# cgtuebingen/3D-RE-GEN

Hardware: NVIDIA H100
Metric: objects->mesh/sec (256^3 SDF, 50 DiT steps) (higher is better)
Workload: dtype f16

## Files before the change

### 3d-re-gen_b200/csrc/attn.cu

```cuda
#include <cuda_fp16.h>
#include <math.h>

#include "r3g_internal.h"
#include "r3g_ptx.cuh"

namespace {

using namespace r3g;

constexpr int kD = 64;
constexpr int kWG = 3;
constexpr int kBQ = 64 * kWG;
constexpr int kBKV = 128;
constexpr int kStg = 3;
constexpr int kQBytes = 64 * kD * 2;
constexpr int kTileBytes = kBKV * kD * 2;
constexpr int kTilesBytes = kQBytes * kWG + 2 * kStg * kTileBytes;
constexpr int kSmemBytes = kTilesBytes + 1024 + 256;
constexpr int kThreads = 128 * kWG + 32;

struct AttnParams {
  __half* o;
  int64_t o_sb, o_sh, o_sl;
  int Lq, Lk;
  float scale_log2;
};

__global__ void __launch_bounds__(kThreads, 1)
attention_kernel(const __grid_constant__ CUtensorMap tmap_q, const __grid_constant__ CUtensorMap tmap_k,
                 const __grid_constant__ CUtensorMap tmap_v, const AttnParams p) {
  extern __shared__ uint8_t smem_raw[];
  uint8_t* smem = reinterpret_cast<uint8_t*>((reinterpret_cast<uintptr_t>(smem_raw) + 1023) & ~(uintptr_t)1023);
  uint8_t* sQ = smem;
  uint8_t* sK = sQ + kWG * kQBytes;
  uint8_t* sV = sK + kStg * kTileBytes;
  uint64_t* q_full = reinterpret_cast<uint64_t*>(smem + kTilesBytes);
  uint64_t* k_full = q_full + 1;
  uint64_t* v_full = k_full + kStg;
  uint64_t* k_empty = v_full + kStg;
  uint64_t* v_empty = k_empty + kStg;

  const int warp = threadIdx.x >> 5;
  const int lane = threadIdx.x & 31;
  const int q0 = blockIdx.x * kBQ;
  const int h = blockIdx.y, b = blockIdx.z;
  const int n_kv = (p.Lk + kBKV - 1) / kBKV;

  if (warp == 4 * kWG && lane == 0) {
    tma_prefetch_desc(&tmap_q);
    tma_prefetch_desc(&tmap_k);
    tma_prefetch_desc(&tmap_v);
    mbar_init(q_full, 1);
    for (int s = 0; s < kStg; ++s) {
      mbar_init(&k_full[s], 1);
      mbar_init(&v_full[s], 1);
      mbar_init(&k_empty[s], 128 * kWG);
      mbar_init(&v_empty[s], 128 * kWG);
    }
    fence_barrier_init();
  }
  __syncthreads();
  pdl_wait();

  if (warp == 4 * kWG) {
    if (lane == 0) {
      const int groups = min(kWG, (p.Lq - q0 + 63) / 64);
      mbar_expect_tx(q_full, groups * kQBytes);
      for (int g = 0; g < groups; ++g) tma_load_4d(sQ + g * kQBytes, &tmap_q, q_full, 0, q0 + 64 * g, h, b, kEvictFirst);
      for (int j = 0; j < n_kv; ++j) {
        const int st = j % kStg;
        const uint32_t ph = (j / kStg) & 1;
        mbar_wait(&k_empty[st], ph ^ 1);
        mbar_expect_tx(&k_full[st], kTileBytes);
        tma_load_4d(sK + st * kTileBytes, &tmap_k, &k_full[st], 0, j * kBKV, h, b, kEvictLast);
        mbar_wait(&v_empty[st], ph ^ 1);
        mbar_expect_tx(&v_full[st], kTileBytes);
        tma_load_4d(sV + st * kTileBytes, &tmap_v, &v_full[st], 0, j * kBKV, h, b, kEvictLast);
      }
    }
    return;
  }

  const int wg = warp >> 2;
  const int r0 = (warp & 3) * 16 + (lane >> 2);
  const int c0 = 2 * (lane & 3);
  const uint32_t aq = smem_u32(sQ + wg * kQBytes);
  float o[kD / 2];
#pragma unroll
  for (int i = 0; i < kD / 2; ++i) o[i] = 0.f;
  float m_run[2] = {-INFINITY, -INFINITY}, l_run[2] = {0.f, 0.f};
  mbar_wait(q_full, 0);
  for (int j = 0; j < n_kv; ++j) {
    const int st = j % kStg;
    const uint32_t ph = (j / kStg) & 1;
    float s[kBKV / 2];
    mbar_wait(&k_full[st], ph);
    const uint32_t ak = smem_u32(sK + st * kTileBytes);
    wgmma_fence();
#pragma unroll
    for (int k = 0; k < kD / 16; ++k)
      wgmma_m64n128k16_ss(s, gmma_desc_sw128(aq + k * 32, 1024, 16), gmma_desc_sw128(ak + k * 32, 1024, 16),
                          k ? 1u : 0u);
    wgmma_commit();
    wgmma_wait<0>();
    wgmma_reg_fence<kBKV / 2>(s);
    mbar_arrive(&k_empty[st]);

    const int valid = min(kBKV, p.Lk - j * kBKV);
    if (valid < kBKV) {
#pragma unroll
      for (int i = 0; i < kBKV / 2; ++i)
        if (8 * (i >> 2) + c0 + (i & 1) >= valid) s[i] = -INFINITY;
    }
    float mx[2] = {-INFINITY, -INFINITY};
#pragma unroll
    for (int i = 0; i < kBKV / 2; ++i) mx[(i >> 1) & 1] = fmaxf(mx[(i >> 1) & 1], s[i]);
    float alpha[2];
#pragma unroll
    for (int rr = 0; rr < 2; ++rr) {
      mx[rr] = fmaxf(mx[rr], __shfl_xor_sync(0xffffffffu, mx[rr], 1));
      mx[rr] = fmaxf(mx[rr], __shfl_xor_sync(0xffffffffu, mx[rr], 2));
      const float m_new = fmaxf(m_run[rr], mx[rr] * p.scale_log2);
      alpha[rr] = ex2_approx(m_run[rr] - m_new);
      m_run[rr] = m_new;
      l_run[rr] *= alpha[rr];
    }
#pragma unroll
    for (int i = 0; i < kD / 2; ++i) o[i] *= alpha[(i >> 1) & 1];
    uint32_t pk[kBKV / 16][4];
#pragma unroll
    for (int i = 0; i < kBKV / 2; i += 2) {
      const int rr = (i >> 1) & 1;
      const float e0 = ex2_approx(fmaf(s[i], p.scale_log2, -m_run[rr]));
      const float e1 = ex2_approx(fmaf(s[i + 1], p.scale_log2, -m_run[rr]));
      l_run[rr] += e0 + e1;
      pk[i >> 3][(i >> 1) & 3] = pack_half2(e0, e1);
    }
    mbar_wait(&v_full[st], ph);
    const uint32_t av = smem_u32(sV + st * kTileBytes);
    wgmma_fence();
#pragma unroll
    for (int k = 0; k < kBKV / 16; ++k) wgmma_m64n64k16_rs_tb(o, pk[k], gmma_desc_sw128(av + k * 2048, 1024, 1024), 1u);
    wgmma_commit();
    wgmma_wait<0>();
    wgmma_reg_fence<kD / 2>(o);
    mbar_arrive(&v_empty[st]);
  }

  float inv_l[2];
#pragma unroll
  for (int rr = 0; rr < 2; ++rr) {
    float l = l_run[rr];
    l += __shfl_xor_sync(0xffffffffu, l, 1);
    l += __shfl_xor_sync(0xffffffffu, l, 2);
    inv_l[rr] = 1.f / l;
  }
#pragma unroll
  for (int rr = 0; rr < 2; ++rr) {
    const int qrow = q0 + wg * 64 + r0 + 8 * rr;
    if (qrow >= p.Lq) continue;
    __half* op = p.o + (int64_t)b * p.o_sb + (int64_t)h * p.o_sh + (int64_t)qrow * p.o_sl;
#pragma unroll
    for (int i = 2 * rr; i < kD / 2; i += 4)
      *reinterpret_cast<uint32_t*>(op + 8 * (i >> 2) + c0) = pack_half2(o[i] * inv_l[rr], o[i + 1] * inv_l[rr]);
  }
}

int make_qkv_map(r3g_ctx* ctx, CUtensorMap* m, const void* base, int64_t sb, int64_t sh, int64_t sl, int B, int H,
                 int L, int box_rows) {
  const uint64_t dims[4] = {(uint64_t)kD, (uint64_t)L, (uint64_t)H, (uint64_t)B};
  const uint64_t strides[4] = {2, (uint64_t)sl * 2, (uint64_t)sh * 2, (uint64_t)sb * 2};
  const uint32_t box[4] = {(uint32_t)kD, (uint32_t)box_rows, 1, 1};
  return r3g_make_tmap_f16(ctx, m, base, 4, dims, strides, box);
}

}

extern "C" int r3g_attention(r3g_ctx* ctx, const r3g_attention_args* a, void* stream) {
  R3G_ENTRY(ctx, "attention");
  if (!a || !a->q || !a->k || !a->v || !a->o) return r3g_fail(ctx, R3G_E_INVALID, "attention: null argument");
  if (a->B < 1 || a->H < 1 || a->Lq < 1 || a->Lk < 1) return r3g_fail(ctx, R3G_E_INVALID, "attention: empty shape");
  if (a->o_sl % 8 || a->o_sh % 8 || a->o_sb % 8 || !r3g_aligned16(a->o))
    return r3g_fail(ctx, R3G_E_INVALID, "attention: output strides must be multiples of 8 halfs");
  CUtensorMap mq, mk, mv;
  int rc;
  if ((rc = make_qkv_map(ctx, &mq, a->q, a->q_sb, a->q_sh, a->q_sl, a->B, a->H, a->Lq, 64))) return rc;
  if ((rc = make_qkv_map(ctx, &mk, a->k, a->k_sb, a->k_sh, a->k_sl, a->B, a->H, a->Lk, kBKV))) return rc;
  if ((rc = make_qkv_map(ctx, &mv, a->v, a->v_sb, a->v_sh, a->v_sl, a->B, a->H, a->Lk, kBKV))) return rc;
  AttnParams p;
  p.o = (__half*)a->o;
  p.o_sb = a->o_sb; p.o_sh = a->o_sh; p.o_sl = a->o_sl;
  p.Lq = a->Lq; p.Lk = a->Lk;
  p.scale_log2 = a->scale * 1.4426950408889634f;
  if (!(ctx->attr_done & R3G_ATTR_ATTENTION)) {
    R3G_CUDA_OK(ctx, cudaFuncSetAttribute(attention_kernel, cudaFuncAttributeMaxDynamicSharedMemorySize, kSmemBytes));
    R3G_CUDA_OK(ctx, cudaFuncSetAttribute(attention_kernel, cudaFuncAttributePreferredSharedMemoryCarveout, 100));
    ctx->attr_done |= R3G_ATTR_ATTENTION;
  }
  dim3 grid((a->Lq + kBQ - 1) / kBQ, a->H, a->B);
  R3G_CUDA_OK(ctx, r3g_launch_pdl(ctx, attention_kernel, grid, dim3(kThreads), kSmemBytes, (cudaStream_t)stream, mq, mk, mv, p));
  R3G_LAUNCH_OK(ctx);
  return R3G_OK;
}
```

### 3d-re-gen_b200/csrc/r3g_ptx.cuh

```cuda
#pragma once
#include <cuda.h>
#include <cuda_fp16.h>
#include <cuda_runtime.h>
#include <stdint.h>

namespace r3g {

__device__ __forceinline__ uint32_t smem_u32(const void* p) {
  return static_cast<uint32_t>(__cvta_generic_to_shared(p));
}

__device__ __forceinline__ bool elect_one() {
  uint32_t pred = 0;
  asm volatile(
      "{\n\t.reg .pred P;\n\t"
      "elect.sync _|P, 0xffffffff;\n\t"
      "selp.u32 %0, 1, 0, P;\n\t}\n"
      : "=r"(pred));
  return pred != 0;
}

__device__ __forceinline__ void mbar_init(uint64_t* bar, uint32_t count) {
  asm volatile("mbarrier.init.shared::cta.b64 [%0], %1;\n" ::"r"(smem_u32(bar)), "r"(count));
}
__device__ __forceinline__ void pdl_wait() { asm volatile("griddepcontrol.wait;" ::: "memory"); }
__device__ __forceinline__ void pdl_trigger() { asm volatile("griddepcontrol.launch_dependents;" ::: "memory"); }

__device__ __forceinline__ void fence_barrier_init() {
  asm volatile("fence.mbarrier_init.release.cluster;\n" ::: "memory");
}
__device__ __forceinline__ void mbar_expect_tx(uint64_t* bar, uint32_t bytes) {
  asm volatile("mbarrier.arrive.expect_tx.shared::cta.b64 _, [%0], %1;\n" ::"r"(smem_u32(bar)), "r"(bytes)
               : "memory");
}
__device__ __forceinline__ void mbar_arrive(uint64_t* bar) {
  asm volatile("mbarrier.arrive.shared::cta.b64 _, [%0];\n" ::"r"(smem_u32(bar)) : "memory");
}
constexpr uint32_t kMbarSuspendHint = 0x989680u;
__device__ __forceinline__ bool mbar_try_wait(uint64_t* bar, uint32_t parity) {
  uint32_t ok;
  asm volatile(
      "{\n\t.reg .pred P;\n\t"
      "mbarrier.try_wait.parity.shared::cta.b64 P, [%1], %2, %3;\n\t"
      "selp.u32 %0, 1, 0, P;\n\t}\n"
      : "=r"(ok)
      : "r"(smem_u32(bar)), "r"(parity), "r"(kMbarSuspendHint)
      : "memory");
  return ok != 0;
}
__device__ __forceinline__ void mbar_wait(uint64_t* bar, uint32_t parity) {
  while (!mbar_try_wait(bar, parity)) {
  }
}

__device__ __forceinline__ void fence_proxy_async_smem() {
  asm volatile("fence.proxy.async.shared::cta;\n" ::: "memory");
}

__device__ __forceinline__ void named_bar_sync(uint32_t id, uint32_t count) {
  asm volatile("bar.sync %0, %1;\n" ::"r"(id), "r"(count) : "memory");
}

__device__ __forceinline__ void tma_prefetch_desc(const CUtensorMap* m) {
  asm volatile("prefetch.tensormap [%0];\n" ::"l"(reinterpret_cast<uint64_t>(m)) : "memory");
}
constexpr uint64_t kEvictNormal = 0x1000000000000000ull;
constexpr uint64_t kEvictFirst = 0x12F0000000000000ull;
constexpr uint64_t kEvictLast = 0x14F0000000000000ull;

__device__ __forceinline__ void tma_load_2d(void* smem_dst, const CUtensorMap* m, uint64_t* bar, int c0, int c1,
                                            uint64_t hint = kEvictNormal) {
  asm volatile(
      "cp.async.bulk.tensor.2d.shared::cluster.global.mbarrier::complete_tx::bytes.L2::cache_hint"
      " [%0], [%1, {%3, %4}], [%2], %5;\n" ::"r"(smem_u32(smem_dst)),
      "l"(reinterpret_cast<uint64_t>(m)), "r"(smem_u32(bar)), "r"(c0), "r"(c1), "l"(hint)
      : "memory");
}
__device__ __forceinline__ void tma_load_3d(void* smem_dst, const CUtensorMap* m, uint64_t* bar, int c0, int c1,
                                            int c2, uint64_t hint = kEvictNormal) {
  asm volatile(
      "cp.async.bulk.tensor.3d.shared::cluster.global.mbarrier::complete_tx::bytes.L2::cache_hint"
      " [%0], [%1, {%3, %4, %5}], [%2], %6;\n" ::"r"(smem_u32(smem_dst)),
      "l"(reinterpret_cast<uint64_t>(m)), "r"(smem_u32(bar)), "r"(c0), "r"(c1), "r"(c2), "l"(hint)
      : "memory");
}
__device__ __forceinline__ void tma_load_4d(void* smem_dst, const CUtensorMap* m, uint64_t* bar, int c0, int c1,
                                            int c2, int c3, uint64_t hint = kEvictNormal) {
  asm volatile(
      "cp.async.bulk.tensor.4d.shared::cluster.global.mbarrier::complete_tx::bytes.L2::cache_hint"
      " [%0], [%1, {%3, %4, %5, %6}], [%2], %7;\n" ::"r"(smem_u32(smem_dst)),
      "l"(reinterpret_cast<uint64_t>(m)), "r"(smem_u32(bar)), "r"(c0), "r"(c1), "r"(c2), "r"(c3), "l"(hint)
      : "memory");
}

__device__ __forceinline__ void wgmma_fence() { asm volatile("wgmma.fence.sync.aligned;\n" ::: "memory"); }
__device__ __forceinline__ void wgmma_commit() { asm volatile("wgmma.commit_group.sync.aligned;\n" ::: "memory"); }
template <int N>
__device__ __forceinline__ void wgmma_wait() {
  asm volatile("wgmma.wait_group.sync.aligned %0;\n" ::"n"(N) : "memory");
}
template <int N>
__device__ __forceinline__ void wgmma_reg_fence(float* d) {
#pragma unroll
  for (int i = 0; i < N; ++i) asm volatile("" : "+f"(d[i])::"memory");
}
__device__ __forceinline__ void wgmma_m64n128k16_ss(float* d, uint64_t desc_a, uint64_t desc_b, uint32_t accumulate) {
  asm volatile(
      "{\n\t.reg .pred p;\n\t"
      "setp.ne.b32 p, %66, 0;\n\t"
      "wgmma.mma_async.sync.aligned.m64n128k16.f32.f16.f16 "
      "{%0, %1, %2, %3, %4, %5, %6, %7, %8, %9, %10, %11, %12, %13, %14, %15, %16, %17, %18, %19, %20, %21, %22, %23, %24, %25, %26, %27, %28, %29, %30, %31, %32, %33, %34, %35, %36, %37, %38, %39, %40, %41, %42, %43, %44, %45, %46, %47, %48, %49, %50, %51, %52, %53, %54, %55, %56, %57, %58, %59, %60, %61, %62, %63}, "
      "%64, %65, p, 1, 1, 0, 0;\n\t}\n"
      : "+f"(d[0]), "+f"(d[1]), "+f"(d[2]), "+f"(d[3]), "+f"(d[4]), "+f"(d[5]), "+f"(d[6]), "+f"(d[7]), "+f"(d[8]), "+f"(d[9]), "+f"(d[10]), "+f"(d[11]), "+f"(d[12]), "+f"(d[13]), "+f"(d[14]), "+f"(d[15]), "+f"(d[16]), "+f"(d[17]), "+f"(d[18]), "+f"(d[19]), "+f"(d[20]), "+f"(d[21]), "+f"(d[22]), "+f"(d[23]), "+f"(d[24]), "+f"(d[25]), "+f"(d[26]), "+f"(d[27]), "+f"(d[28]), "+f"(d[29]), "+f"(d[30]), "+f"(d[31]), "+f"(d[32]), "+f"(d[33]), "+f"(d[34]), "+f"(d[35]), "+f"(d[36]), "+f"(d[37]), "+f"(d[38]), "+f"(d[39]), "+f"(d[40]), "+f"(d[41]), "+f"(d[42]), "+f"(d[43]), "+f"(d[44]), "+f"(d[45]), "+f"(d[46]), "+f"(d[47]), "+f"(d[48]), "+f"(d[49]), "+f"(d[50]), "+f"(d[51]), "+f"(d[52]), "+f"(d[53]), "+f"(d[54]), "+f"(d[55]), "+f"(d[56]), "+f"(d[57]), "+f"(d[58]), "+f"(d[59]), "+f"(d[60]), "+f"(d[61]), "+f"(d[62]), "+f"(d[63])
      : "l"(desc_a), "l"(desc_b), "r"(accumulate));
}
__device__ __forceinline__ void wgmma_m64n256k16_ss(float* d, uint64_t desc_a, uint64_t desc_b, uint32_t accumulate) {
  asm volatile(
      "{\n\t.reg .pred p;\n\t"
      "setp.ne.b32 p, %130, 0;\n\t"
      "wgmma.mma_async.sync.aligned.m64n256k16.f32.f16.f16 "
      "{%0, %1, %2, %3, %4, %5, %6, %7, %8, %9, %10, %11, %12, %13, %14, %15, %16, %17, %18, %19, %20, %21, %22, %23, %24, %25, %26, %27, %28, %29, %30, %31, %32, %33, %34, %35, %36, %37, %38, %39, %40, %41, %42, %43, %44, %45, %46, %47, %48, %49, %50, %51, %52, %53, %54, %55, %56, %57, %58, %59, %60, %61, %62, %63, %64, %65, %66, %67, %68, %69, %70, %71, %72, %73, %74, %75, %76, %77, %78, %79, %80, %81, %82, %83, %84, %85, %86, %87, %88, %89, %90, %91, %92, %93, %94, %95, %96, %97, %98, %99, %100, %101, %102, %103, %104, %105, %106, %107, %108, %109, %110, %111, %112, %113, %114, %115, %116, %117, %118, %119, %120, %121, %122, %123, %124, %125, %126, %127}, "
      "%128, %129, p, 1, 1, 0, 0;\n\t}\n"
      : "+f"(d[0]), "+f"(d[1]), "+f"(d[2]), "+f"(d[3]), "+f"(d[4]), "+f"(d[5]), "+f"(d[6]), "+f"(d[7]), "+f"(d[8]), "+f"(d[9]), "+f"(d[10]), "+f"(d[11]), "+f"(d[12]), "+f"(d[13]), "+f"(d[14]), "+f"(d[15]), "+f"(d[16]), "+f"(d[17]), "+f"(d[18]), "+f"(d[19]), "+f"(d[20]), "+f"(d[21]), "+f"(d[22]), "+f"(d[23]), "+f"(d[24]), "+f"(d[25]), "+f"(d[26]), "+f"(d[27]), "+f"(d[28]), "+f"(d[29]), "+f"(d[30]), "+f"(d[31]), "+f"(d[32]), "+f"(d[33]), "+f"(d[34]), "+f"(d[35]), "+f"(d[36]), "+f"(d[37]), "+f"(d[38]), "+f"(d[39]), "+f"(d[40]), "+f"(d[41]), "+f"(d[42]), "+f"(d[43]), "+f"(d[44]), "+f"(d[45]), "+f"(d[46]), "+f"(d[47]), "+f"(d[48]), "+f"(d[49]), "+f"(d[50]), "+f"(d[51]), "+f"(d[52]), "+f"(d[53]), "+f"(d[54]), "+f"(d[55]), "+f"(d[56]), "+f"(d[57]), "+f"(d[58]), "+f"(d[59]), "+f"(d[60]), "+f"(d[61]), "+f"(d[62]), "+f"(d[63]), "+f"(d[64]), "+f"(d[65]), "+f"(d[66]), "+f"(d[67]), "+f"(d[68]), "+f"(d[69]), "+f"(d[70]), "+f"(d[71]), "+f"(d[72]), "+f"(d[73]), "+f"(d[74]), "+f"(d[75]), "+f"(d[76]), "+f"(d[77]), "+f"(d[78]), "+f"(d[79]), "+f"(d[80]), "+f"(d[81]), "+f"(d[82]), "+f"(d[83]), "+f"(d[84]), "+f"(d[85]), "+f"(d[86]), "+f"(d[87]), "+f"(d[88]), "+f"(d[89]), "+f"(d[90]), "+f"(d[91]), "+f"(d[92]), "+f"(d[93]), "+f"(d[94]), "+f"(d[95]), "+f"(d[96]), "+f"(d[97]), "+f"(d[98]), "+f"(d[99]), "+f"(d[100]), "+f"(d[101]), "+f"(d[102]), "+f"(d[103]), "+f"(d[104]), "+f"(d[105]), "+f"(d[106]), "+f"(d[107]), "+f"(d[108]), "+f"(d[109]), "+f"(d[110]), "+f"(d[111]), "+f"(d[112]), "+f"(d[113]), "+f"(d[114]), "+f"(d[115]), "+f"(d[116]), "+f"(d[117]), "+f"(d[118]), "+f"(d[119]), "+f"(d[120]), "+f"(d[121]), "+f"(d[122]), "+f"(d[123]), "+f"(d[124]), "+f"(d[125]), "+f"(d[126]), "+f"(d[127])
      : "l"(desc_a), "l"(desc_b), "r"(accumulate));
}
__device__ __forceinline__ void wgmma_m64n64k16_rs_tb(float* d, const uint32_t* a, uint64_t desc_b, uint32_t accumulate) {
  asm volatile(
      "{\n\t.reg .pred p;\n\t"
      "setp.ne.b32 p, %37, 0;\n\t"
      "wgmma.mma_async.sync.aligned.m64n64k16.f32.f16.f16 "
      "{%0, %1, %2, %3, %4, %5, %6, %7, %8, %9, %10, %11, %12, %13, %14, %15, %16, %17, %18, %19, %20, %21, %22, %23, %24, %25, %26, %27, %28, %29, %30, %31}, "
      "{%32, %33, %34, %35}, %36, p, 1, 1, 1;\n\t}\n"
      : "+f"(d[0]), "+f"(d[1]), "+f"(d[2]), "+f"(d[3]), "+f"(d[4]), "+f"(d[5]), "+f"(d[6]), "+f"(d[7]), "+f"(d[8]), "+f"(d[9]), "+f"(d[10]), "+f"(d[11]), "+f"(d[12]), "+f"(d[13]), "+f"(d[14]), "+f"(d[15]), "+f"(d[16]), "+f"(d[17]), "+f"(d[18]), "+f"(d[19]), "+f"(d[20]), "+f"(d[21]), "+f"(d[22]), "+f"(d[23]), "+f"(d[24]), "+f"(d[25]), "+f"(d[26]), "+f"(d[27]), "+f"(d[28]), "+f"(d[29]), "+f"(d[30]), "+f"(d[31])
      : "r"(a[0]), "r"(a[1]), "r"(a[2]), "r"(a[3]), "l"(desc_b), "r"(accumulate));
}
__device__ __forceinline__ uint64_t f2_pack(float lo, float hi) {
  uint64_t r;
  asm("mov.b64 %0, {%1, %2};" : "=l"(r) : "f"(lo), "f"(hi));
  return r;
}
__device__ __forceinline__ void f2_unpack(uint64_t v, float& lo, float& hi) {
  asm("mov.b64 {%0, %1}, %2;" : "=f"(lo), "=f"(hi) : "l"(v));
}
__device__ __forceinline__ uint64_t f2_fma(uint64_t a, uint64_t b, uint64_t c) {
  float a0, a1, b0, b1, c0, c1;
  f2_unpack(a, a0, a1); f2_unpack(b, b0, b1); f2_unpack(c, c0, c1);
  return f2_pack(__fmaf_rn(a0, b0, c0), __fmaf_rn(a1, b1, c1));
}
__device__ __forceinline__ uint64_t f2_add(uint64_t a, uint64_t b) {
  float a0, a1, b0, b1;
  f2_unpack(a, a0, a1); f2_unpack(b, b0, b1);
  return f2_pack(__fadd_rn(a0, b0), __fadd_rn(a1, b1));
}
__device__ __forceinline__ uint64_t f2_mul(uint64_t a, uint64_t b) {
  float a0, a1, b0, b1;
  f2_unpack(a, a0, a1); f2_unpack(b, b0, b1);
  return f2_pack(__fmul_rn(a0, b0), __fmul_rn(a1, b1));
}
__device__ __forceinline__ uint32_t f2_to_h2(uint64_t v) {
  float lo, hi;
  f2_unpack(v, lo, hi);
  uint32_t r;
  asm("cvt.rn.f16x2.f32 %0, %1, %2;" : "=r"(r) : "f"(hi), "f"(lo));
  return r;
}
__device__ __forceinline__ uint64_t h2_to_f2(uint32_t h) {
  const float2 f = __half22float2(*reinterpret_cast<const __half2*>(&h));
  return f2_pack(f.x, f.y);
}

__device__ __forceinline__ uint64_t gmma_desc_sw128(uint32_t saddr, uint32_t sbo_bytes, uint32_t lbo_bytes) {
  uint64_t d = 0;
  d |= (uint64_t)((saddr & 0x3FFFF) >> 4);
  d |= (uint64_t)((lbo_bytes >> 4) & 0x3FFF) << 16;
  d |= (uint64_t)((sbo_bytes >> 4) & 0x3FFF) << 32;
  d |= (uint64_t)1 << 62;
  return d;
}

__device__ __forceinline__ uint32_t pack_half2(float a, float b) {
  __half2 h = __floats2half2_rn(a, b);
  return *reinterpret_cast<uint32_t*>(&h);
}
__device__ __forceinline__ float h2f(__half h) { return __half2float(h); }
__device__ __forceinline__ float rnd_h(float x) { return __half2float(__float2half_rn(x)); }

struct alignas(16) Half8 {
  uint4 u;
};
__device__ __forceinline__ void unpack8(const Half8 p, float* f) {
  const __half2* v = reinterpret_cast<const __half2*>(&p.u);
#pragma unroll
  for (int i = 0; i < 4; ++i) {
    float2 t = __half22float2(v[i]);
    f[2 * i] = t.x;
    f[2 * i + 1] = t.y;
  }
}
__device__ __forceinline__ Half8 pack8(const float* f) {
  Half8 p;
  __half2* v = reinterpret_cast<__half2*>(&p.u);
#pragma unroll
  for (int i = 0; i < 4; ++i) v[i] = __floats2half2_rn(f[2 * i], f[2 * i + 1]);
  return p;
}

__device__ __forceinline__ float warp_sum(float v) {
#pragma unroll
  for (int o = 16; o > 0; o >>= 1) v += __shfl_xor_sync(0xffffffffu, v, o);
  return v;
}
__device__ __forceinline__ float ex2_approx(float x) {
  float y;
  asm("ex2.approx.ftz.f32 %0, %1;" : "=f"(y) : "f"(x));
  return y;
}

}
```

Measured before the change: 0.2632.

## Overlap next QK^T with current PV wgmma and rebalance registers via setmaxnreg

The attention consumer loop is restructured so the S=QK^T wgmma for the next KV tile is issued together with the PV wgmma of the current tile. Softmax for the next tile then runs while PV is still in flight, instead of serialising score GEMM, softmax and PV. The producer is widened to a full warpgroup so setmaxnreg can shift registers from it to the consumer warpgroups, which need room for two score tiles and the accumulator. The output rescale by alpha is skipped when a warp sees no change in the running max. The cost is more register pressure and a more complex pipeline prologue and epilogue.

```diff
diff --git a/3d-re-gen_b200/csrc/attn.cu b/3d-re-gen_b200/csrc/attn.cu
--- a/3d-re-gen_b200/csrc/attn.cu
+++ b/3d-re-gen_b200/csrc/attn.cu
@@ -17,7 +17,9 @@
 constexpr int kTileBytes = kBKV * kD * 2;
 constexpr int kTilesBytes = kQBytes * kWG + 2 * kStg * kTileBytes;
 constexpr int kSmemBytes = kTilesBytes + 1024 + 256;
-constexpr int kThreads = 128 * kWG + 32;
+constexpr int kThreads = 128 * (kWG + 1);
+constexpr uint32_t kProducerRegs = 24, kConsumerRegs = 160;
+static_assert(kWG * 128 * kConsumerRegs + 128 * kProducerRegs <= 65536, "register file of one SM");
 
 struct AttnParams {
   __half* o;
@@ -25,6 +27,38 @@
   int Lq, Lk;
   float scale_log2;
 };
+
+__device__ __forceinline__ void online_softmax(float (&s)[kBKV / 2], float (&m_run)[2], float (&l_run)[2],
+                                               float (&alpha)[2], int valid, int c0, float scale_log2) {
+  if (valid < kBKV) {
+#pragma unroll
+    for (int i = 0; i < kBKV / 2; ++i)
+      if (8 * (i >> 2) + c0 + (i & 1) >= valid) s[i] = -INFINITY;
+  }
+  float mx[2] = {-INFINITY, -INFINITY};
+#pragma unroll
+  for (int i = 0; i < kBKV / 2; ++i) mx[(i >> 1) & 1] = fmaxf(mx[(i >> 1) & 1], s[i]);
+#pragma unroll
+  for (int rr = 0; rr < 2; ++rr) {
+    mx[rr] = fmaxf(mx[rr], __shfl_xor_sync(0xffffffffu, mx[rr], 1));
+    mx[rr] = fmaxf(mx[rr], __shfl_xor_sync(0xffffffffu, mx[rr], 2));
+    const float m_new = fmaxf(m_run[rr], mx[rr] * scale_log2);
+    alpha[rr] = ex2_approx(m_run[rr] - m_new);
+    m_run[rr] = m_new;
+    l_run[rr] *= alpha[rr];
+  }
+#pragma unroll
+  for (int i = 0; i < kBKV / 2; i += 2) {
+    const int rr = (i >> 1) & 1;
+    s[i] = ex2_approx(fmaf(s[i], scale_log2, -m_run[rr]));
+    s[i + 1] = ex2_approx(fmaf(s[i + 1], scale_log2, -m_run[rr]));
+    l_run[rr] += s[i] + s[i + 1];
+  }
+}
+__device__ __forceinline__ void pack_p(const float (&s)[kBKV / 2], uint32_t (&pk)[kBKV / 16][4]) {
+#pragma unroll
+  for (int i = 0; i < kBKV / 2; i += 2) pk[i >> 3][(i >> 1) & 3] = pack_half2(s[i], s[i + 1]);
+}
 
 __global__ void __launch_bounds__(kThreads, 1)
 attention_kernel(const __grid_constant__ CUtensorMap tmap_q, const __grid_constant__ CUtensorMap tmap_k,
@@ -62,8 +96,9 @@
   __syncthreads();
   pdl_wait();
 
-  if (warp == 4 * kWG) {
-    if (lane == 0) {
+  if (warp >= 4 * kWG) {
+    setmaxnreg_dec<kProducerRegs>();
+    if (warp == 4 * kWG && lane == 0) {
       const int groups = min(kWG, (p.Lq - q0 + 63) / 64);
       mbar_expect_tx(q_full, groups * kQBytes);
       for (int g = 0; g < groups; ++g) tma_load_4d(sQ + g * kQBytes, &tmap_q, q_full, 0, q0 + 64 * g, h, b, kEvictFirst);
@@ -81,6 +116,7 @@
     return;
   }
 
+  setmaxnreg_inc<kConsumerRegs>();
   const int wg = warp >> 2;
   const int r0 = (warp & 3) * 16 + (lane >> 2);
   const int c0 = 2 * (lane & 3);
@@ -88,13 +124,12 @@
   float o[kD / 2];
 #pragma unroll
   for (int i = 0; i < kD / 2; ++i) o[i] = 0.f;
-  float m_run[2] = {-INFINITY, -INFINITY}, l_run[2] = {0.f, 0.f};
-  mbar_wait(q_full, 0);
-  for (int j = 0; j < n_kv; ++j) {
+  float m_run[2] = {-INFINITY, -INFINITY}, l_run[2] = {0.f, 0.f}, alpha[2];
+  uint32_t pk[kBKV / 16][4];
+
+  auto issue_s = [&](float (&s)[kBKV / 2], int j) {
     const int st = j % kStg;
-    const uint32_t ph = (j / kStg) & 1;
-    float s[kBKV / 2];
-    mbar_wait(&k_full[st], ph);
+    mbar_wait(&k_full[st], (j / kStg) & 1);
     const uint32_t ak = smem_u32(sK + st * kTileBytes);
     wgmma_fence();
 #pragma unroll
@@ -102,50 +137,51 @@
       wgmma_m64n128k16_ss(s, gmma_desc_sw128(aq + k * 32, 1024, 16), gmma_desc_sw128(ak + k * 32, 1024, 16),
                           k ? 1u : 0u);
     wgmma_commit();
+  };
+  auto issue_pv = [&](int j) {
+    const int st = j % kStg;
+    mbar_wait(&v_full[st], (j / kStg) & 1);
+    const uint32_t av = smem_u32(sV + st * kTileBytes);
+    wgmma_fence();
+#pragma unroll
+    for (int k = 0; k < kBKV / 16; ++k) wgmma_m64n64k16_rs_tb(o, pk[k], gmma_desc_sw128(av + k * 2048, 1024, 1024), 1u);
+    wgmma_commit();
+  };
+  auto retire_pv = [&](int j) {
+    wgmma_wait<0>();
+    wgmma_reg_fence<kD / 2>(o);
+    mbar_arrive(&v_empty[j % kStg]);
+  };
+
+  mbar_wait(q_full, 0);
+  {
+    float s[kBKV / 2];
+    issue_s(s, 0);
     wgmma_wait<0>();
     wgmma_reg_fence<kBKV / 2>(s);
-    mbar_arrive(&k_empty[st]);
-
-    const int valid = min(kBKV, p.Lk - j * kBKV);
-    if (valid < kBKV) {
-#pragma unroll
-      for (int i = 0; i < kBKV / 2; ++i)
-        if (8 * (i >> 2) + c0 + (i & 1) >= valid) s[i] = -INFINITY;
+    mbar_arrive(&k_empty[0]);
+    online_softmax(s, m_run, l_run, alpha, min(kBKV, p.Lk), c0, p.scale_log2);
+    pack_p(s, pk);
+  }
+  for (int j = 0; j + 1 < n_kv; ++j) {
+    float s[kBKV / 2];
+    issue_s(s, j + 1);
+    issue_pv(j);
+    wgmma_wait<1>();
+    wgmma_reg_fence<kBKV / 2>(s);
+    mbar_arrive(&k_empty[(j + 1) % kStg]);
+    online_softmax(s, m_run, l_run, alpha, min(kBKV, p.Lk - (j + 1) * kBKV), c0, p.scale_log2);
+    if (__all_sync(0xffffffffu, alpha[0] == 1.f && alpha[1] == 1.f)) {
+      retire_pv(j);
+    } else {
+      retire_pv(j);
+#pragma unroll
+      for (int i = 0; i < kD / 2; ++i) o[i] *= alpha[(i >> 1) & 1];
     }
-    float mx[2] = {-INFINITY, -INFINITY};
-#pragma unroll
-    for (int i = 0; i < kBKV / 2; ++i) mx[(i >> 1) & 1] = fmaxf(mx[(i >> 1) & 1], s[i]);
-    float alpha[2];
-#pragma unroll
-    for (int rr = 0; rr < 2; ++rr) {
-      mx[rr] = fmaxf(mx[rr], __shfl_xor_sync(0xffffffffu, mx[rr], 1));
-      mx[rr] = fmaxf(mx[rr], __shfl_xor_sync(0xffffffffu, mx[rr], 2));
-      const float m_new = fmaxf(m_run[rr], mx[rr] * p.scale_log2);
-      alpha[rr] = ex2_approx(m_run[rr] - m_new);
-      m_run[rr] = m_new;
-      l_run[rr] *= alpha[rr];
-    }
-#pragma unroll
-    for (int i = 0; i < kD / 2; ++i) o[i] *= alpha[(i >> 1) & 1];
-    uint32_t pk[kBKV / 16][4];
-#pragma unroll
-    for (int i = 0; i < kBKV / 2; i += 2) {
-      const int rr = (i >> 1) & 1;
-      const float e0 = ex2_approx(fmaf(s[i], p.scale_log2, -m_run[rr]));
-      const float e1 = ex2_approx(fmaf(s[i + 1], p.scale_log2, -m_run[rr]));
-      l_run[rr] += e0 + e1;
-      pk[i >> 3][(i >> 1) & 3] = pack_half2(e0, e1);
-    }
-    mbar_wait(&v_full[st], ph);
-    const uint32_t av = smem_u32(sV + st * kTileBytes);
-    wgmma_fence();
-#pragma unroll
-    for (int k = 0; k < kBKV / 16; ++k) wgmma_m64n64k16_rs_tb(o, pk[k], gmma_desc_sw128(av + k * 2048, 1024, 1024), 1u);
-    wgmma_commit();
-    wgmma_wait<0>();
-    wgmma_reg_fence<kD / 2>(o);
-    mbar_arrive(&v_empty[st]);
-  }
+    pack_p(s, pk);
+  }
+  issue_pv(n_kv - 1);
+  retire_pv(n_kv - 1);
 
   float inv_l[2];
 #pragma unroll
diff --git a/3d-re-gen_b200/csrc/r3g_ptx.cuh b/3d-re-gen_b200/csrc/r3g_ptx.cuh
--- a/3d-re-gen_b200/csrc/r3g_ptx.cuh
+++ b/3d-re-gen_b200/csrc/r3g_ptx.cuh
@@ -59,6 +59,15 @@
 
 __device__ __forceinline__ void named_bar_sync(uint32_t id, uint32_t count) {
   asm volatile("bar.sync %0, %1;\n" ::"r"(id), "r"(count) : "memory");
+}
+
+template <uint32_t N>
+__device__ __forceinline__ void setmaxnreg_dec() {
+  asm volatile("setmaxnreg.dec.sync.aligned.u32 %0;\n" ::"n"(N));
+}
+template <uint32_t N>
+__device__ __forceinline__ void setmaxnreg_inc() {
+  asm volatile("setmaxnreg.inc.sync.aligned.u32 %0;\n" ::"n"(N));
 }
 
 __device__ __forceinline__ void tma_prefetch_desc(const CUtensorMap* m) {
```

After: 0.2671, median of 6. 1.01x the previous value.
